# luisdiaz1997/GPzoo

Measured on AMD Instinct MI355X. Metric: ELBO evals/sec (L=32-latent evaluations, all GPUs) at M=2048 inducing, N=200000, L=32 latents/GPU x 1 GPU(s), higher is better.
Workload: dtype f32; 1 GPU; BASELINE configs[2]: Slide-seq-shaped synthetic, N=200000 spots, M=2048, L=32 latents/GPU x 1 GPU(s), matern32, f32; latents_total=32, whitened=True, chunk=0, factor_dtype=f64

## Files before the change

gpzoo_amd/csrc/gemmw.h:

```cpp
#pragma once
#include "common.h"

namespace gpz {

struct Fused1Args {
  const float* Linv; int64_t Mp;
  const float* Z; int64_t M;
  const float* X; int64_t nreal;
  int d, kind, L;
  const float* sigma; const float* ell;
  float* Wt; int64_t ncp;
  const float* muE;
  float* ps_sq; float* ps_mu;
};
bool fused1_supported(int dtype, int kind, int d);
int fused1_launch(const Fused1Args& a, hipStream_t s);

enum WideEpilogue {
  WIDE_STORE_STATS = 0,
  WIDE_STATS = 1,
  WIDE_STORE = 2,
  WIDE_STORE_COLSCALE = 3,
  WIDE_WBAR = 4,
  WIDE_KBAR = 5,
  WIDE_ADD_COLSCALE = 6,
};
struct WideArgs {
  const float* A; const float* B; int64_t Mp, ncp; int L;
  int upper, epilogue;
  float* C; const float* mu;
  float* ps_sq; float* ps_mu;
  const float* colscale; const float* colvec;
  const float* rowvec;
  const float* aux;
  const int32_t* gate;
};
bool wide_product_supported(int64_t Mp, int64_t ncp);
int wide_product_launch(const WideArgs& a, hipStream_t s);

bool wide_nt_supported(int64_t Mp, int64_t K);
int wide_nt_pieces(int64_t Mp, int64_t K, int L);
size_t wide_nt_scratch_floats(int64_t Mp, int64_t K, int L);
size_t wide_nt_vpart_floats(int64_t Mp, int64_t K, int L);
int wide_nt_launch(const float* A, const float* B, float* C, int64_t Mp, int64_t K, int L, hipStream_t s, float* scratch = nullptr,
                   const float* w = nullptr, const int32_t* gate = nullptr, const float* gm = nullptr, float* vpart = nullptr,
                   double* v = nullptr, int64_t v_stride = 0);

}
```

gpzoo_amd/csrc/gemmw.hip:

```cpp
#include "gemmw.h"

#include "cov.h"


#include <cmath>
#include <mutex>
#include <type_traits>
#include <utility>

#ifndef GPZ_W_ABL
#define GPZ_W_ABL 0
#endif

namespace gpz {

typedef float f32x4 __attribute__((ext_vector_type(4)));

enum { WB_MEM = 0, WB_GEN = 1 };
enum { WA_DENSE = 0, WA_LOWER = 1, WA_UPPER = 2 };
enum { WE_STORE_STATS = 0,
       WE_STATS = 1,
       WE_STORE = 2,
       WE_STORE_COLSCALE = 3,
       WE_WBAR = 4,
       WE_KBAR = 5,
       WE_ADD_COLSCALE = 6 };

struct WParams {
  const float* A; int64_t lda, sA0;
  const float* B; int64_t ldb, sB0;
  const float* Z; int64_t MD;
  const float* X; int64_t nreal;
  const float* sigma; const float* ell;
  float* C; int64_t ldc, sC0;
  const float* mu; int64_t sMu;
  float* ps_sq; float* ps_mu; int64_t ncols;
  const float* colscale; const float* colvec; int64_t sCs;
  const float* rowvec; int64_t sRv;
  const float* aux;
  int64_t M;
  int L, nblk, mtw, nt, W, strips;
  int pair, colmajor;
  const int32_t* gate;
};

constexpr int W_BK = 16;

template <int TM, int TN, int BSRC, int D>
struct WLds {
  static constexpr int A_ELEMS = TM * W_BK;
  static constexpr int RPP = 256 / TN;
  static constexpr int PITCH = 256 + (RPP == 2 ? 8 : RPP == 1 ? 4 : 16);
  static constexpr int B_ELEMS = (W_BK / RPP) * PITCH;
  static constexpr int STAGE = A_ELEMS + B_ELEMS;
  static constexpr int ZB = 128 * D;
  static constexpr size_t bytes = sizeof(float) * (2 * STAGE + (BSRC == WB_GEN ? 2 * ZB : 0));
};

template <int TM, int TN, int BSRC, int ATRI, int EPI, int KIND, int D>
__global__ __launch_bounds__(64 * (TM / 128) * (TN / 32)) __attribute__((amdgpu_waves_per_eu(4, 4))) void gemmw_kernel(const WParams p) {
  constexpr int BK = W_BK;
  if (p.gate && *p.gate == 0) return;
  constexpr int WMW = TM / 128, WNW = TN / 32;
  constexpr int NW = WMW * WNW;
  static_assert(NW == 8 || NW == 16, "8 or 16 waves of 128 x 32");
  using G = WLds<TM, TN, BSRC, D>;
  constexpr int RPP = G::RPP, PITCH = G::PITCH;
  extern __shared__ __attribute__((aligned(1024))) char smem_raw[];
  float* const smem = reinterpret_cast<float*>(smem_raw);
  auto sA = [&](int buf) -> float* { return smem + buf * G::STAGE; };
  auto sB = [&](int buf) -> float* { return smem + buf * G::STAGE + G::A_ELEMS; };
  float* const sZ = smem + 2 * G::STAGE;
  auto addrB = [](int k, int n) { return (k / RPP) * PITCH + (k % RPP) * TN + n; };

  int tj, b0, leg_ti[2], nlegs = 1;
  {
    const int bid = blockIdx.x;
    const int x = bid & 7, s = bid >> 3;
    if (BSRC == WB_GEN) {
      const int ug = s / p.W, within = s - ug * p.W;
      const int u = ug * 8 + x;
      const int per_level = p.L * p.strips;
      if (u >= p.mtw * per_level) return;
      const int level = u / per_level, rem = u - level * per_level;
      leg_ti[0] = leg_ti[1] = (ATRI == WA_LOWER) ? p.mtw - 1 - level : level;
      b0 = rem / p.strips;
      tj = (rem - b0 * p.strips) * p.W + within;
    } else {
// ... 257 lines not shown
        for (int g = 0; g < 4; ++g)
#pragma unroll
          for (int ni = 0; ni < 2; ++ni) {
            const float v = acc[mi][ni][g];
            ssq[ni] = __builtin_fmaf(v, v, ssq[ni]);
            if constexpr (EPI == WE_STORE_STATS) smu[ni] = __builtin_fmaf(m4[g], v, smu[ni]);
          }
      }
#pragma unroll
      for (int ni = 0; ni < 2; ++ni) {
        ssq[ni] += __shfl_xor(ssq[ni], 16); ssq[ni] += __shfl_xor(ssq[ni], 32);
        if constexpr (EPI == WE_STORE_STATS) { smu[ni] += __shfl_xor(smu[ni], 16); smu[ni] += __shfl_xor(smu[ni], 32); }
        if (q == 0) {
          const int64_t o = ((int64_t)b0 * p.nblk + db) * p.ncols + ccol0 + ni * 16 + r;
          p.ps_sq[o] = ssq[ni];
          if constexpr (EPI == WE_STORE_STATS) p.ps_mu[o] = smu[ni];
        }
      }
    }
    if constexpr (EPI != WE_STATS) {
      constexpr int LDE = 36;
      static_assert(NW * 16 * LDE <= G::STAGE, "the epilogue strips fit tile buffer 1");
      float* strip = sA(1) + wave * (16 * LDE);
      float* Cg = p.C + b0 * p.sC0 + row0 * p.ldc + ccol0;
      int srow = lane >> 3;
      asm volatile("" : "+v"(srow));
      const int c4 = (lane & 7) * 4;
      float cs[2] = {1.f, 1.f};
      if constexpr (EPI == WE_STORE_COLSCALE) {
#pragma unroll
        for (int ni = 0; ni < 2; ++ni) cs[ni] = p.colscale[b0 * p.sCs + ccol0 + ni * 16 + r];
      }
      f32x4 sc = {0, 0, 0, 0}, cv = {0, 0, 0, 0};
      if constexpr (EPI == WE_WBAR || EPI == WE_KBAR || EPI == WE_ADD_COLSCALE)
        sc = *reinterpret_cast<const f32x4*>(p.colscale + b0 * p.sCs + ccol0 + c4);
      if constexpr (EPI == WE_WBAR || EPI == WE_KBAR)
        cv = *reinterpret_cast<const f32x4*>(p.colvec + b0 * p.sCs + ccol0 + c4);
#pragma unroll
      for (int mi = 0; mi < 8; ++mi) {
#pragma unroll
        for (int ni = 0; ni < 2; ++ni)
#pragma unroll
          for (int g = 0; g < 4; ++g) strip[(4 * q + g) * LDE + ni * 16 + r] = cs[ni] * acc[mi][ni][g];
        __builtin_amdgcn_wave_barrier();
        f32x4 w[2];
        float rv[2];
        if constexpr (EPI == WE_WBAR || EPI == WE_KBAR || EPI == WE_ADD_COLSCALE) {
#pragma unroll
          for (int it = 0; it < 2; ++it) {
            const int64_t row = mi * 16 + it * 8 + srow;
            if constexpr (EPI == WE_WBAR) w[it] = *reinterpret_cast<const f32x4*>(p.aux + b0 * p.sC0 + (row0 + row) * p.ldc + ccol0 + c4);
            if constexpr (EPI == WE_ADD_COLSCALE) w[it] = *reinterpret_cast<const f32x4*>(Cg + (int64_t)row * p.ldc + c4);
            if constexpr (EPI != WE_ADD_COLSCALE) rv[it] = p.rowvec[b0 * p.sRv + row0 + row];
          }
        }
#pragma unroll
        for (int it = 0; it < 2; ++it) {
          const int row = it * 8 + srow;
          f32x4 v = *reinterpret_cast<const f32x4*>(strip + row * LDE + c4);
          if constexpr (EPI == WE_WBAR) {
#pragma unroll
            for (int e = 0; e < 4; ++e) v[e] = v[e] + rv[it] * cv[e] - w[it][e] * sc[e];
          }
          if constexpr (EPI == WE_KBAR) {
#pragma unroll
            for (int e = 0; e < 4; ++e) v[e] = v[e] * sc[e] + rv[it] * cv[e];
          }
          if constexpr (EPI == WE_ADD_COLSCALE) {
#pragma unroll
            for (int e = 0; e < 4; ++e) v[e] = w[it][e] + v[e] * sc[e];
          }
          *reinterpret_cast<f32x4*>(Cg + (int64_t)(mi * 16 + row) * p.ldc + c4) = v;
        }
        __builtin_amdgcn_wave_barrier();
      }
    }
  }
}

struct NTParams {
  const float* A; const float* B; float* C;
  int64_t ld, sAB, ldc, sC;
  int K, nblk, mt, L, T;
  int S, Ks;
  float* part; int64_t sPart;
  const float* w; int64_t sW;
  const int32_t* gate;
  const float* gm; float* vpart;
};

template <int TM, bool WTS>
__global__ __launch_bounds__(TM * 2) __attribute__((amdgpu_waves_per_eu(4, 4))) void gemmw_nt_kernel(const NTParams p) {
  constexpr int BK = W_BK, TN = 128;
  if (p.gate && *p.gate == 0) return;
  constexpr int NW = TM / 32;
  constexpr int A_ELEMS = TM * BK, B_ELEMS = TN * BK, STAGE = A_ELEMS + B_ELEMS;
  extern __shared__ __attribute__((aligned(1024))) char smem_raw[];
  float* const smem = reinterpret_cast<float*>(smem_raw);
  auto sA = [&](int buf) -> float* { return smem + buf * STAGE; };
  auto sB = [&](int buf) -> float* { return smem + buf * STAGE + A_ELEMS; };
  int b0, ti, tj, piece;
  {
    const int nb = (int)gridDim.x, qn = nb >> 3, rem = nb & 7, x = blockIdx.x & 7;
    const int lid0 = x * qn + min(x, rem) + (int)(blockIdx.x >> 3);
    const int grp = lid0 / p.T;
    const int t = lid0 - grp * p.T;
    b0 = grp / p.S;
    piece = grp - b0 * p.S;
    if constexpr (TM == 256) {
      int i = (int)((sqrtf(4.0f * (float)t + 1.0f) - 1.0f) * 0.5f);
      while ((i + 1) * (i + 2) <= t) ++i;
      while (i * (i + 1) > t) --i;
      ti = i; tj = t - i * (i + 1);
    } else {
      int i = (int)((sqrtf(8.0f * (float)t + 1.0f) - 1.0f) * 0.5f);
      while ((i + 1) * (i + 2) / 2 <= t) ++i;
      while (i * (i + 1) / 2 > t) --i;
      ti = i; tj = t - i * (i + 1) / 2;
    }
  }
  const int tid = threadIdx.x, lane = tid & 63;
  const int wave = __builtin_amdgcn_readfirstlane(tid >> 6);
  const int wm = wave >> 2, wn = wave & 3;
  const int r = lane & 15, q = lane >> 4;
  const int Mp = p.nblk * 128;
  const int db = (TM / 128) * ti + wm;
  const bool active = db < p.nblk && tj <= db;
  const bool same = TM == 128 && p.A == p.B && tj == ti;
  typedef __attribute__((address_space(3))) void lds_void;
#if defined(__HIP_DEVICE_COMPILE__)
  const __amdgpu_buffer_rsrc_t a_rsrc = __builtin_amdgcn_make_buffer_rsrc(
      const_cast<float*>(p.A + b0 * p.sAB), 0, (int)(p.ld * Mp * sizeof(float)), 0x00020000);
  const __amdgpu_buffer_rsrc_t b_rsrc = __builtin_amdgcn_make_buffer_rsrc(
      const_cast<float*>(p.B + b0 * p.sAB), 0, (int)(p.ld * Mp * sizeof(float)), 0x00020000);
#endif
  auto gperm = [](int w) { const int t = (w >> 2) & 3; return (((t >> 1) ^ t) & 1) << 1 | (t >> 1); };
  const int voff = ((lane >> 2) * (int)p.ld + (((lane & 3) ^ gperm(lane >> 2)) * 4)) * (int)sizeof(float);
  int a_soff[2], b_soff;
#pragma unroll
  for (int h = 0; h < 2; ++h) {
    int row = ti * TM + (2 * wave + h) * 16;
    while (row >= Mp) row -= 128;
    a_soff[h] = (row * (int)p.ld + piece * p.Ks) * (int)sizeof(float);
  }
  constexpr int NPB = 8 / NW;
  b_soff = ((tj * TN + wave * NPB * 16) * (int)p.ld + piece * p.Ks) * (int)sizeof(float);
  auto stage_load = [&](int buf) __attribute__((always_inline)) {
#if defined(__HIP_DEVICE_COMPILE__)
#pragma unroll
    for (int h = 0; h < 2; ++h) {
      __builtin_amdgcn_raw_ptr_buffer_load_lds(a_rsrc, (lds_void*)(sA(buf) + (2 * wave + h) * 256), 16, voff, a_soff[h], 0, 0);
      a_soff[h] += BK * (int)sizeof(float);
    }
    if (!same) {
#pragma unroll
      for (int h = 0; h < NPB; ++h)
        __builtin_amdgcn_raw_ptr_buffer_load_lds(b_rsrc, (lds_void*)(sB(buf) + (wave * NPB + h) * 256), 16, voff,
                                                 b_soff + h * 16 * (int)p.ld * (int)sizeof(float), 0, 0);
      b_soff += BK * (int)sizeof(float);
    }
#endif
  };
  const float* wk = WTS ? p.w + b0 * p.sW + (int64_t)piece * p.Ks + 4 * (lane >> 4) : nullptr;
  f32x4 wv;
  auto w_load = [&]() __attribute__((always_inline)) {
    if constexpr (WTS) { wv = *reinterpret_cast<const f32x4*>(wk); wk += BK; }
  };
  const int fr_a = (wm * 128 + r) * BK + ((q ^ gperm(r)) * 4);
  const int nk = (min(p.K, (piece + 1) * p.Ks) - piece * p.Ks) / BK;
  const bool split = p.S > 1;
  const bool diag = WTS && p.A == p.B && db == tj && db < p.nblk;
  if (diag) {
    auto diag_path = [&](auto wn_c) __attribute__((always_inline)) {
      constexpr int C0 = decltype(wn_c)::value, C1 = 7 - C0, N0 = 8 - C0, N1 = 8 - C1;
      const bool rd = p.gm != nullptr;
      const float* gk = rd ? p.gm + b0 * p.sW + (int64_t)piece * p.Ks + 4 * (lane >> 4) : nullptr;
      f32x4 gv = f32x4{0, 0, 0, 0};
      float pv0 = 0.f, pv1 = 0.f;
      f32x4 a0[N0], a1[N1];
#pragma unroll
      for (int i = 0; i < N0; ++i) a0[i] = f32x4{0, 0, 0, 0};
#pragma unroll
      for (int i = 0; i < N1; ++i) a1[i] = f32x4{0, 0, 0, 0};
      const int fb_off = r * BK + ((q ^ gperm(r)) * 4) + (same ? -A_ELEMS : 0);
      auto step = [&](int buf, bool more) __attribute__((always_inline)) {
        f32x4 f0 = *reinterpret_cast<const f32x4*>(sB(buf) + fb_off + C0 * 16 * BK);
        f32x4 f1 = *reinterpret_cast<const f32x4*>(sB(buf) + fb_off + C1 * 16 * BK);
        f0 *= wv; f1 *= wv;
        if (more) w_load();
#pragma unroll
        for (int mi = C0; mi < 8; ++mi) {
          const f32x4 fa = *reinterpret_cast<const f32x4*>(sA(buf) + fr_a + mi * 16 * BK);
#pragma unroll
          for (int j = 0; j < 4; ++j) {
            a0[mi - C0] = __builtin_amdgcn_mfma_f32_16x16x4f32(fa[j], f0[j], a0[mi - C0], 0, 0, 0);
            if (mi >= C1) a1[mi >= C1 ? mi - C1 : 0] = __builtin_amdgcn_mfma_f32_16x16x4f32(fa[j], f1[j], a1[mi >= C1 ? mi - C1 : 0], 0, 0, 0);
          }
          if (mi == 2 * C0 || mi == 2 * C0 + 1) {
            if (rd) {
              const f32x4 t = fa * gv;
              if (mi == 2 * C0) pv0 += (t[0] + t[1]) + (t[2] + t[3]); else pv1 += (t[0] + t[1]) + (t[2] + t[3]);
            }
          }
        }
        if (more && rd) { gv = *reinterpret_cast<const f32x4*>(gk); gk += BK; }
      };
      if (rd) { gv = *reinterpret_cast<const f32x4*>(gk); gk += BK; }
      stage_load(0);
      w_load();
      asm volatile("s_waitcnt vmcnt(0)" ::: "memory");
      __syncthreads();
      for (int t = 0; t < nk; t += 2) {
        if (t + 1 < nk) stage_load(1);
        step(0, t + 1 < nk);
        asm volatile("s_waitcnt vmcnt(0)" ::: "memory");
        __syncthreads();
        if (t + 2 < nk) stage_load(0);
        step(1, t + 2 < nk);
        asm volatile("s_waitcnt vmcnt(0)" ::: "memory");
        __syncthreads();
      }
      if (rd) {
        float* vp = p.vpart + ((int64_t)piece * p.L + b0) * Mp + db * 128;
        pv0 += __shfl_xor(pv0, 16); pv0 += __shfl_xor(pv0, 32);
        pv1 += __shfl_xor(pv1, 16); pv1 += __shfl_xor(pv1, 32);
        if (q == 0) { vp[(2 * C0) * 16 + r] = pv0; vp[(2 * C0 + 1) * 16 + r] = pv1; }
      }
      float* Cg = (split ? p.part + piece * p.sPart : p.C) + b0 * p.sC + (int64_t)db * 128 * p.ldc + (int64_t)tj * TN;
      auto put = [&](const f32x4& a, int mi, int c) __attribute__((always_inline)) {
        float* o = Cg + (int64_t)(mi * 16 + 4 * q) * p.ldc + c * 16 + r;
#pragma unroll
        for (int g = 0; g < 4; ++g) o[g * p.ldc] = split ? a[g] : o[g * p.ldc] + a[g];
      };
#pragma unroll
      for (int mi = C0; mi < 8; ++mi) put(a0[mi - C0], mi, C0);
#pragma unroll
      for (int mi = C1; mi < 8; ++mi) put(a1[mi - C1], mi, C1);
    };
    switch (wn) {
      case 0: diag_path(std::integral_constant<int, 0>{}); break;
      case 1: diag_path(std::integral_constant<int, 1>{}); break;
      case 2: diag_path(std::integral_constant<int, 2>{}); break;
      default: diag_path(std::integral_constant<int, 3>{}); break;
    }
    return;
  }
  f32x4 acc[8][2];
#pragma unroll
  for (int mi = 0; mi < 8; ++mi)
#pragma unroll
    for (int ni = 0; ni < 2; ++ni) acc[mi][ni] = f32x4{0, 0, 0, 0};
  const int fr_b = (wn * 32 + r) * BK + ((q ^ gperm(r)) * 4) + (same ? -A_ELEMS : 0);
  auto mma_step = [&](int buf, bool more) __attribute__((always_inline)) {
    f32x4 fb[2];
#pragma unroll
    for (int ni = 0; ni < 2; ++ni) {
      fb[ni] = *reinterpret_cast<const f32x4*>(sB(buf) + fr_b + ni * 16 * BK);
      if constexpr (WTS) fb[ni] *= wv;
    }
    if (more) w_load();
#pragma unroll
    for (int half = 0; half < 2; ++half) {
      f32x4 fa[4];
#pragma unroll
      for (int m = 0; m < 4; ++m) fa[m] = *reinterpret_cast<const f32x4*>(sA(buf) + fr_a + (half * 4 + m) * 16 * BK);
#pragma unroll
      for (int j = 0; j < 4; ++j)
#pragma unroll
        for (int m = 0; m < 4; ++m)
#pragma unroll
          for (int ni = 0; ni < 2; ++ni)
            acc[half * 4 + m][ni] = __builtin_amdgcn_mfma_f32_16x16x4f32(fa[m][j], fb[ni][j], acc[half * 4 + m][ni], 0, 0, 0);
    }
  };
  stage_load(0);
  w_load();
  asm volatile("s_waitcnt vmcnt(0)" ::: "memory");
  __syncthreads();
  if (active) {
    for (int t = 0; t < nk; t += 2) {
      if (t + 1 < nk) stage_load(1);
      mma_step(0, t + 1 < nk);
      asm volatile("s_waitcnt vmcnt(0)" ::: "memory");
      __syncthreads();
      if (t + 2 < nk) stage_load(0);
      mma_step(1, t + 2 < nk);
      asm volatile("s_waitcnt vmcnt(0)" ::: "memory");
      __syncthreads();
    }
  } else {
    for (int t = 0; t < nk; t += 2) {
      if (t + 1 < nk) stage_load(1);
      asm volatile("s_waitcnt vmcnt(0)" ::: "memory");
      __syncthreads();
      if (t + 2 < nk) stage_load(0);
      asm volatile("s_waitcnt vmcnt(0)" ::: "memory");
      __syncthreads();
    }
    return;
  }
  constexpr int LDE = 36;
  float* strip = smem + wave * (32 * LDE);
  float* Cg = (split ? p.part + piece * p.sPart : p.C) + b0 * p.sC + (int64_t)db * 128 * p.ldc + (int64_t)tj * TN + wn * 32;
  const int srow = lane >> 3, c4 = (lane & 7) * 4;
#pragma unroll
  for (int pass = 0; pass < 4; ++pass) {
#pragma unroll
    for (int mm = 0; mm < 2; ++mm)
#pragma unroll
      for (int ni = 0; ni < 2; ++ni)
#pragma unroll
        for (int g = 0; g < 4; ++g) strip[(mm * 16 + 4 * q + g) * LDE + ni * 16 + r] = acc[pass * 2 + mm][ni][g];
    __builtin_amdgcn_wave_barrier();
    f32x4 cin[4];
#pragma unroll
    for (int it = 0; it < 4; ++it)
      cin[it] = split ? f32x4{0, 0, 0, 0} : *reinterpret_cast<const f32x4*>(Cg + (int64_t)(pass * 32 + it * 8 + srow) * p.ldc + c4);
#pragma unroll
    for (int it = 0; it < 4; ++it) {
      const int row = it * 8 + srow;
      const f32x4 v = *reinterpret_cast<const f32x4*>(strip + row * LDE + c4);
      *reinterpret_cast<f32x4*>(Cg + (int64_t)(pass * 32 + row) * p.ldc + c4) = cin[it] + v;
    }
    __builtin_amdgcn_wave_barrier();
  }
}
// ... 64 lines not shown
  p.L = a.L; p.nblk = (int)(a.Mp / 128); p.mtw = (int)((a.Mp + TM - 1) / TM); p.nt = (int)(a.ncp / TN);
  int strips = (p.nt + 31) / 32;
  const int want = (32 + p.mtw * p.L - 1) / (p.mtw * p.L);
  if (strips < want) strips = want < p.nt ? want : p.nt;
  p.W = (p.nt + strips - 1) / strips;
  p.strips = (p.nt + p.W - 1) / p.W;
  const int64_t units = (int64_t)p.mtw * p.L * p.strips;
  const int64_t nblocks = (units + 7) / 8 * 8 * p.W;
#define GPZ_W1(KIND, D) return launch_wide(gemmw_kernel<TM, TN, WB_GEN, WA_LOWER, WE_STORE_STATS, KIND, D>, \
                                           WLds<TM, TN, WB_GEN, D>::bytes, p, nblocks, s, 1024)
  if (a.kind == GPZ_KERNEL_MATERN32) { if (a.d == 2) GPZ_W1(1, 2); GPZ_W1(1, 1); }
  if (a.kind == GPZ_KERNEL_MATERN12) { if (a.d == 2) GPZ_W1(4, 2); GPZ_W1(4, 1); }
  if (a.kind == GPZ_KERNEL_MATERN52) { if (a.d == 2) GPZ_W1(5, 2); GPZ_W1(5, 1); }
  if (a.d == 2) GPZ_W1(0, 2);
  GPZ_W1(0, 1);
#undef GPZ_W1
}

bool wide_product_supported(int64_t Mp, int64_t ncp) {
  return Mp % 128 == 0 && ncp % 128 == 0 && Mp * Mp * 4 < (1ll << 31) && Mp * ncp * 4 < (1ll << 31);
}

template <int TM, int TN>
static int wide_product_launch_t(const WideArgs& a, hipStream_t s) {
  WParams p = {};
  p.A = a.A; p.lda = a.Mp; p.sA0 = a.Mp * a.Mp;
  p.B = a.B; p.ldb = a.ncp; p.sB0 = a.Mp * a.ncp;
  p.C = a.C; p.ldc = a.ncp; p.sC0 = a.Mp * a.ncp;
  p.mu = a.mu; p.sMu = a.Mp;
  p.ps_sq = a.ps_sq; p.ps_mu = a.ps_mu; p.ncols = a.ncp; p.M = a.Mp;
  p.colscale = a.colscale; p.colvec = a.colvec; p.sCs = a.ncp; p.rowvec = a.rowvec; p.sRv = a.Mp; p.aux = a.aux;
  p.gate = a.gate;
  p.L = a.L; p.nblk = (int)(a.Mp / 128); p.mtw = (int)((a.Mp + TM - 1) / TM); p.nt = (int)((a.ncp + TN - 1) / TN);
  constexpr int WMAX = 4096 / TN;
  int strips = (p.nt + WMAX - 1) / WMAX;
  const int want = (8 + p.L - 1) / p.L;
  if (strips < want) strips = want < p.nt ? want : p.nt;
  p.strips = strips;
  p.W = (p.nt + strips - 1) / strips;
  const int64_t units = (int64_t)p.L * p.strips;
  const int64_t paired = (units + 7) / 8 * 8 * ((p.mtw + 1) / 2) * p.W;
  p.pair = p.colmajor = paired >= 4 * 512;
  const int64_t nblocks = p.pair ? paired : (units + 7) / 8 * 8 * p.mtw * p.W;
  constexpr size_t lds = WLds<TM, TN, WB_MEM, 1>::bytes;
#define GPZ_WM(ATRI, EPI) return launch_wide(gemmw_kernel<TM, TN, WB_MEM, ATRI, EPI, 0, 1>, lds, p, nblocks, s)
  switch (a.epilogue) {
    case WIDE_STORE_STATS:
      GPZ_REQUIRE(!a.upper && a.C && a.mu && a.ps_sq && a.ps_mu, "wide product: store + statistics is the lower-triangular product and needs C, mu and both slabs");
      GPZ_WM(WA_LOWER, WE_STORE_STATS);
    case WIDE_STATS:
      GPZ_REQUIRE(a.upper && a.ps_sq, "wide product: statistics only is the upper-triangular product");
      GPZ_WM(WA_UPPER, WE_STATS);
    case WIDE_STORE:
      GPZ_REQUIRE(a.upper && a.C, "wide product: the plain store is built for the upper-triangular product");
      GPZ_WM(WA_UPPER, WE_STORE);
    case WIDE_STORE_COLSCALE:
      GPZ_REQUIRE(a.upper && a.C && a.colscale, "wide product: the column-scaled store is the upper-triangular product and needs the factors");
      GPZ_WM(WA_UPPER, WE_STORE_COLSCALE);
    case WIDE_WBAR:
      GPZ_REQUIRE(!a.upper && a.C && a.colscale && a.colvec && a.rowvec && a.aux, "wide product: the W-bar epilogue needs its operands");
      GPZ_WM(WA_LOWER, WE_WBAR);
    case WIDE_KBAR:
      GPZ_REQUIRE(a.upper == 2 && a.C && a.colscale && a.colvec && a.rowvec, "wide product: the K-bar epilogue is the dense product and needs its vectors");
      GPZ_WM(WA_DENSE, WE_KBAR);
    case WIDE_ADD_COLSCALE:
      GPZ_REQUIRE(a.upper == 1 && a.C && a.colscale, "wide product: the accumulating column-scaled store is the upper-triangular product");
      GPZ_WM(WA_UPPER, WE_ADD_COLSCALE);
    default: break;
  }
#undef GPZ_WM
  GPZ_REQUIRE(false, "wide product: unknown epilogue %d", a.epilogue);
}

int wide_product_launch(const WideArgs& a, hipStream_t s) {
  GPZ_REQUIRE(wide_product_supported(a.Mp, a.ncp) && a.L > 0, "wide product: bad extents");
  return wide_product_launch_t<128, 256>(a, s);
}

bool wide_nt_supported(int64_t Mp, int64_t K) {
  return Mp % 128 == 0 && K % 128 == 0 && K > 0 && Mp * K * 4 < (1ll << 31);
}

static bool nt_small_tiles(int64_t nblk) { return nblk <= 4; }
static int64_t nt_tiles(int64_t nblk) {
  if (nt_small_tiles(nblk)) return nblk * (nblk + 1) / 2;
  const int64_t mt = (nblk + 1) / 2;
  return mt * (mt + 1) - (nblk & 1);
}

int wide_nt_pieces(int64_t Mp, int64_t K, int L) {
  const int64_t tiles = nt_tiles(Mp / 128) * L;
  if (tiles >= 384) {
    const double r = (double)tiles / 512.0;
    int best = 1;
    double best_cost = 1e30;
    for (int S = 1; S <= 4; ++S) {
      if (S > 1 && K / S < 2048) break;
      const double rounds = r * S, cost = std::ceil(rounds - 1e-9) / rounds * (1.0 + 0.015 * (S - 1));
      if (cost < best_cost - 1e-9) { best_cost = cost; best = S; }
    }
    return best;
  }
  int64_t S = (nt_small_tiles(Mp / 128) ? 1024 : 512) / tiles;
  S = std::min<int64_t>(S, K / 1024);
  S = std::min<int64_t>(S, 16);
  return (int)std::max<int64_t>(S, 1);
}

size_t wide_nt_vpart_floats(int64_t Mp, int64_t K, int L) { return (size_t)wide_nt_pieces(Mp, K, L) * L * Mp; }

size_t wide_nt_scratch_floats(int64_t Mp, int64_t K, int L) {
  const int S = wide_nt_pieces(Mp, K, L);
  return S > 1 ? (size_t)S * L * Mp * Mp : 0;
}

int wide_nt_launch(const float* A, const float* B, float* C, int64_t Mp, int64_t K, int L, hipStream_t s, float* scratch,
                   const float* w, const int32_t* gate, const float* gm, float* vpart, double* v, int64_t v_stride) {
  GPZ_REQUIRE(A && B && C && wide_nt_supported(Mp, K) && L > 0, "wide A B^T: bad arguments");
  GPZ_REQUIRE(!gm || (w && vpart && v && A == B), "wide A B^T: the row products A gm need weights, A == B and their buffers");
  NTParams p;
  p.w = w; p.sW = K; p.gate = gate; p.gm = gm; p.vpart = vpart;
  p.A = A; p.B = B; p.C = C; p.ld = K; p.sAB = Mp * K; p.ldc = Mp; p.sC = Mp * Mp;
  p.K = (int)K; p.nblk = (int)(Mp / 128); p.mt = (p.nblk + 1) / 2; p.L = L;
  const bool small = nt_small_tiles(p.nblk);
  p.T = (int)nt_tiles(p.nblk);
  int S = scratch ? wide_nt_pieces(Mp, K, L) : 1;
  p.Ks = (int)(((K + S - 1) / S + 31) / 32 * 32);
  S = (int)((K + p.Ks - 1) / p.Ks);
  p.S = S; p.part = scratch; p.sPart = (int64_t)L * Mp * Mp;
  const int64_t nblocks = (int64_t)p.T * L * S;
  GPZ_REQUIRE(nblocks > 0 && nblocks < (1ll << 31), "wide A B^T: bad grid");
  if (small) {
    constexpr size_t lds = sizeof(float) * 2 * (128 + 128) * W_BK;
    if (w) hipLaunchKernelGGL((gemmw_nt_kernel<128, true>), dim3((unsigned)nblocks), dim3(256), lds, s, p);
    else hipLaunchKernelGGL((gemmw_nt_kernel<128, false>), dim3((unsigned)nblocks), dim3(256), lds, s, p);
  } else {
    constexpr size_t lds = sizeof(float) * 2 * (256 + 128) * W_BK;
    if (w) hipLaunchKernelGGL((gemmw_nt_kernel<256, true>), dim3((unsigned)nblocks), dim3(512), lds, s, p);
    else hipLaunchKernelGGL((gemmw_nt_kernel<256, false>), dim3((unsigned)nblocks), dim3(512), lds, s, p);
  }
  GPZ_LAUNCH_OK();
  if (S > 1) {
    const int64_t total4 = (int64_t)L * Mp * Mp / 4;
    hipLaunchKernelGGL(nt_reduce_kernel, dim3((unsigned)((total4 + 255) / 256)), dim3(256), 0, s, C, scratch, S, p.sPart, (int)Mp, total4, gate, (int)(w != nullptr && A == B));
    GPZ_LAUNCH_OK();
  }
  if (gm) {
    const int64_t LM = (int64_t)L * Mp;
    hipLaunchKernelGGL(nt_vsum_kernel, dim3((unsigned)((LM + 255) / 256)), dim3(256), 0, s, vpart, S, LM, v, Mp, v_stride);
    GPZ_LAUNCH_OK();
  }
  return 0;
}

}
```

Measured before the change: 2.637 ELBO evals/s.

## Add symmetric diagonal-tile schedule for weighted A·Aᵀ wide NT kernel

For the weighted symmetric case (A == B with weights) on large tiles, the grid now schedules mt*mt tiles. Each diagonal 256-row tile is computed by one block that loads only A and forms the lower triangle of the 256x256 block, where the old schedule used separate 256x128 tiles. This avoids redundant B loads and the upper-triangle MFMA work on diagonal blocks, and changes the split-K piece count to match the new tile count. It adds a large per-wave specialized path that raises register pressure, and the old schedule stays available through an environment variable.

```diff
diff --git a/gpzoo_amd/csrc/gemmw.h b/gpzoo_amd/csrc/gemmw.h
--- a/gpzoo_amd/csrc/gemmw.h
+++ b/gpzoo_amd/csrc/gemmw.h
@@ -39,7 +39,7 @@
 int wide_product_launch(const WideArgs& a, hipStream_t s);
 
 bool wide_nt_supported(int64_t Mp, int64_t K);
-int wide_nt_pieces(int64_t Mp, int64_t K, int L);
+int wide_nt_pieces(int64_t Mp, int64_t K, int L, bool sym = false);
 size_t wide_nt_scratch_floats(int64_t Mp, int64_t K, int L);
 size_t wide_nt_vpart_floats(int64_t Mp, int64_t K, int L);
 int wide_nt_launch(const float* A, const float* B, float* C, int64_t Mp, int64_t K, int L, hipStream_t s, float* scratch = nullptr,
diff --git a/gpzoo_amd/csrc/gemmw.hip b/gpzoo_amd/csrc/gemmw.hip
--- a/gpzoo_amd/csrc/gemmw.hip
+++ b/gpzoo_amd/csrc/gemmw.hip
@@ -4,6 +4,8 @@
 
 
 #include <cmath>
+#include <cstdlib>
+#include <cstring>
 #include <mutex>
 #include <type_traits>
 #include <utility>
@@ -432,6 +434,7 @@
   const float* w; int64_t sW;
   const int32_t* gate;
   const float* gm; float* vpart;
+  int dtiles;
 };
 
 template <int TM, bool WTS>
@@ -445,6 +448,7 @@
   auto sA = [&](int buf) -> float* { return smem + buf * STAGE; };
   auto sB = [&](int buf) -> float* { return smem + buf * STAGE + A_ELEMS; };
   int b0, ti, tj, piece;
+  bool dtile = false;
   {
     const int nb = (int)gridDim.x, qn = nb >> 3, rem = nb & 7, x = blockIdx.x & 7;
     const int lid0 = x * qn + min(x, rem) + (int)(blockIdx.x >> 3);
@@ -452,7 +456,18 @@
     const int t = lid0 - grp * p.T;
     b0 = grp / p.S;
     piece = grp - b0 * p.S;
-    if constexpr (TM == 256) {
+    if (TM == 256 && WTS && p.dtiles) {
+      if (t < p.mt) {
+        ti = t; tj = 2 * t;
+        dtile = 2 * t + 1 < p.nblk;
+      } else {
+        const int u = t - p.mt;
+        int i = (int)((sqrtf(4.0f * (float)u + 1.0f) + 1.0f) * 0.5f);
+        while (i * (i + 1) <= u) ++i;
+        while (i * (i - 1) > u) --i;
+        ti = i; tj = u - i * (i - 1);
+      }
+    } else if constexpr (TM == 256) {
       int i = (int)((sqrtf(4.0f * (float)t + 1.0f) - 1.0f) * 0.5f);
       while ((i + 1) * (i + 2) <= t) ++i;
       while (i * (i + 1) > t) --i;
@@ -497,7 +512,7 @@
       __builtin_amdgcn_raw_ptr_buffer_load_lds(a_rsrc, (lds_void*)(sA(buf) + (2 * wave + h) * 256), 16, voff, a_soff[h], 0, 0);
       a_soff[h] += BK * (int)sizeof(float);
     }
-    if (!same) {
+    if (!same && !dtile) {
 #pragma unroll
       for (int h = 0; h < NPB; ++h)
         __builtin_amdgcn_raw_ptr_buffer_load_lds(b_rsrc, (lds_void*)(sB(buf) + (wave * NPB + h) * 256), 16, voff,
@@ -506,14 +521,121 @@
     }
 #endif
   };
-  const float* wk = WTS ? p.w + b0 * p.sW + (int64_t)piece * p.Ks + 4 * (lane >> 4) : nullptr;
+  const float* wk = WTS ? p.w + b0 * p.sW + (int64_t)piece * p.Ks : nullptr;
+  const unsigned klane = 4 * (unsigned)(lane >> 4);
   f32x4 wv;
   auto w_load = [&]() __attribute__((always_inline)) {
-    if constexpr (WTS) { wv = *reinterpret_cast<const f32x4*>(wk); wk += BK; }
+    if constexpr (WTS) { wv = *reinterpret_cast<const f32x4*>(wk + klane); wk += BK; }
   };
   const int fr_a = (wm * 128 + r) * BK + ((q ^ gperm(r)) * 4);
   const int nk = (min(p.K, (piece + 1) * p.Ks) - piece * p.Ks) / BK;
   const bool split = p.S > 1;
+  if constexpr (TM == 256 && WTS) {
+    if (dtile) {
+      auto dtile_path = [&](auto w_c) __attribute__((always_inline)) {
+        constexpr int C0 = decltype(w_c)::value, C1 = 15 - C0, N0 = 16 - C0, N1 = 16 - C1;
+        const bool rd = p.gm != nullptr;
+        const float* gk = rd ? p.gm + b0 * p.sW + (int64_t)piece * p.Ks : nullptr;
+        f32x4 gv = f32x4{0, 0, 0, 0};
+        float pv0 = 0.f, pv1 = 0.f;
+        f32x4 a0[N0], a1[N1];
+#pragma unroll
+        for (int i = 0; i < N0; ++i) a0[i] = f32x4{0, 0, 0, 0};
+#pragma unroll
+        for (int i = 0; i < N1; ++i) a1[i] = f32x4{0, 0, 0, 0};
+        const int fr = r * BK + ((q ^ gperm(r)) * 4);
+        auto step = [&](int buf, bool more) __attribute__((always_inline)) {
+          f32x4 f0 = *reinterpret_cast<const f32x4*>(sA(buf) + fr + C0 * 16 * BK);
+          f32x4 f1 = *reinterpret_cast<const f32x4*>(sA(buf) + fr + C1 * 16 * BK);
+          f0 *= wv; f1 *= wv;
+          if (more) w_load();
+#pragma unroll
+          for (int mi = C0; mi < 16; ++mi) {
+            const f32x4 fa = *reinterpret_cast<const f32x4*>(sA(buf) + fr + mi * 16 * BK);
+#pragma unroll
+            for (int j = 0; j < 4; ++j) {
+              a0[mi - C0] = __builtin_amdgcn_mfma_f32_16x16x4f32(fa[j], f0[j], a0[mi - C0], 0, 0, 0);
+              if (mi >= C1) a1[mi >= C1 ? mi - C1 : 0] = __builtin_amdgcn_mfma_f32_16x16x4f32(fa[j], f1[j], a1[mi >= C1 ? mi - C1 : 0], 0, 0, 0);
+            }
+            if (mi == 2 * C0 || mi == 2 * C0 + 1) {
+              if (rd) {
+                const f32x4 t = fa * gv;
+                if (mi == 2 * C0) pv0 += (t[0] + t[1]) + (t[2] + t[3]); else pv1 += (t[0] + t[1]) + (t[2] + t[3]);
+              }
+            }
+          }
+          if (more && rd) { gv = *reinterpret_cast<const f32x4*>(gk + klane); gk += BK; }
+        };
+        if (rd) { gv = *reinterpret_cast<const f32x4*>(gk + klane); gk += BK; }
+        stage_load(0);
+        w_load();
+        asm volatile("s_waitcnt vmcnt(0)" ::: "memory");
+        __syncthreads();
+        for (int t = 0; t < nk; t += 2) {
+          if (t + 1 < nk) stage_load(1);
+          step(0, t + 1 < nk);
+          asm volatile("s_waitcnt vmcnt(0)" ::: "memory");
+          __syncthreads();
+          if (t + 2 < nk) stage_load(0);
+          step(1, t + 2 < nk);
+          asm volatile("s_waitcnt vmcnt(0)" ::: "memory");
+          __syncthreads();
+        }
+        if (rd) {
+          float* vp = p.vpart + ((int64_t)piece * p.L + b0) * Mp + ti * 256;
+          pv0 += __shfl_xor(pv0, 16); pv0 += __shfl_xor(pv0, 32);
+          pv1 += __shfl_xor(pv1, 16); pv1 += __shfl_xor(pv1, 32);
+          if (q == 0) { vp[(2 * C0) * 16 + r] = pv0; vp[(2 * C0 + 1) * 16 + r] = pv1; }
+        }
+#if defined(__HIP_DEVICE_COMPILE__)
+        const __amdgpu_buffer_rsrc_t c_rsrc = __builtin_amdgcn_make_buffer_rsrc(
+            (split ? p.part + piece * p.sPart : p.C) + b0 * p.sC, 0, (int)(p.ldc * Mp * sizeof(float)), 0x00020000);
+        const int ldcb = (int)p.ldc * (int)sizeof(float);
+        const int lo = 4 * q * ldcb + r * (int)sizeof(float);
+        const int so = ti * 256 * ldcb + ti * 256 * (int)sizeof(float);
+        auto put_col = [&](const f32x4* a, auto c_c, auto split_c) __attribute__((always_inline)) {
+          constexpr int CC = decltype(c_c)::value;
+#pragma unroll
+          for (int m0 = CC; m0 < 16; m0 += 4) {
+            float cin[4][4];
+#pragma unroll
+            for (int m = 0; m < 4; ++m)
+#pragma unroll
+              for (int g = 0; g < 4; ++g)
+                if (!decltype(split_c)::value && m0 + m < 16)
+                  cin[m][g] = __builtin_bit_cast(float, __builtin_amdgcn_raw_buffer_load_b32(c_rsrc, lo, so + ((m0 + m) * 16 + g) * ldcb + CC * 64, 0));
+#pragma unroll
+            for (int m = 0; m < 4; ++m)
+#pragma unroll
+              for (int g = 0; g < 4; ++g)
+                if (m0 + m < 16) {
+                  const float v = decltype(split_c)::value ? a[m0 + m - CC][g] : cin[m][g] + a[m0 + m - CC][g];
+                  __builtin_amdgcn_raw_buffer_store_b32(__builtin_bit_cast(unsigned, v), c_rsrc, lo, so + ((m0 + m) * 16 + g) * ldcb + CC * 64, 0);
+                }
+          }
+        };
+        if (split) {
+          put_col(a0, std::integral_constant<int, C0>{}, std::true_type{});
+          put_col(a1, std::integral_constant<int, C1>{}, std::true_type{});
+        } else {
+          put_col(a0, std::integral_constant<int, C0>{}, std::false_type{});
+          put_col(a1, std::integral_constant<int, C1>{}, std::false_type{});
+        }
+#endif
+      };
+      switch (wave) {
+        case 0: dtile_path(std::integral_constant<int, 0>{}); break;
+        case 1: dtile_path(std::integral_constant<int, 1>{}); break;
+        case 2: dtile_path(std::integral_constant<int, 2>{}); break;
+        case 3: dtile_path(std::integral_constant<int, 3>{}); break;
+        case 4: dtile_path(std::integral_constant<int, 4>{}); break;
+        case 5: dtile_path(std::integral_constant<int, 5>{}); break;
+        case 6: dtile_path(std::integral_constant<int, 6>{}); break;
+        default: dtile_path(std::integral_constant<int, 7>{}); break;
+      }
+      return;
+    }
+  }
   const bool diag = WTS && p.A == p.B && db == tj && db < p.nblk;
   if (diag) {
     auto diag_path = [&](auto wn_c) __attribute__((always_inline)) {
@@ -817,14 +939,22 @@
 }
 
 static bool nt_small_tiles(int64_t nblk) { return nblk <= 4; }
-static int64_t nt_tiles(int64_t nblk) {
+
+static bool nt_diag_tiles() {
+  const char* e = getenv("GPZ_NT_SCHEDULE");
+  return !(e && !strcmp(e, "blocks"));
+}
+
+static bool nt_sym_tiles(int64_t nblk, bool sym) { return sym && !nt_small_tiles(nblk) && nt_diag_tiles(); }
+static int64_t nt_tiles(int64_t nblk, bool sym_tiles) {
   if (nt_small_tiles(nblk)) return nblk * (nblk + 1) / 2;
   const int64_t mt = (nblk + 1) / 2;
+  if (sym_tiles) return mt * mt;
   return mt * (mt + 1) - (nblk & 1);
 }
 
-int wide_nt_pieces(int64_t Mp, int64_t K, int L) {
-  const int64_t tiles = nt_tiles(Mp / 128) * L;
+int wide_nt_pieces(int64_t Mp, int64_t K, int L, bool sym) {
+  const int64_t tiles = nt_tiles(Mp / 128, nt_sym_tiles(Mp / 128, sym)) * L;
   if (tiles >= 384) {
     const double r = (double)tiles / 512.0;
     int best = 1;
@@ -842,10 +972,12 @@
   return (int)std::max<int64_t>(S, 1);
 }
 
-size_t wide_nt_vpart_floats(int64_t Mp, int64_t K, int L) { return (size_t)wide_nt_pieces(Mp, K, L) * L * Mp; }
+static int nt_pieces_max(int64_t Mp, int64_t K, int L) { return std::max(wide_nt_pieces(Mp, K, L, false), wide_nt_pieces(Mp, K, L, true)); }
+
+size_t wide_nt_vpart_floats(int64_t Mp, int64_t K, int L) { return (size_t)nt_pieces_max(Mp, K, L) * L * Mp; }
 
 size_t wide_nt_scratch_floats(int64_t Mp, int64_t K, int L) {
-  const int S = wide_nt_pieces(Mp, K, L);
+  const int S = nt_pieces_max(Mp, K, L);
   return S > 1 ? (size_t)S * L * Mp * Mp : 0;
 }
 
@@ -858,8 +990,10 @@
   p.A = A; p.B = B; p.C = C; p.ld = K; p.sAB = Mp * K; p.ldc = Mp; p.sC = Mp * Mp;
   p.K = (int)K; p.nblk = (int)(Mp / 128); p.mt = (p.nblk + 1) / 2; p.L = L;
   const bool small = nt_small_tiles(p.nblk);
-  p.T = (int)nt_tiles(p.nblk);
-  int S = scratch ? wide_nt_pieces(Mp, K, L) : 1;
+  const bool sym = w && A == B;
+  p.dtiles = nt_sym_tiles(p.nblk, sym);
+  p.T = (int)nt_tiles(p.nblk, p.dtiles);
+  int S = scratch ? wide_nt_pieces(Mp, K, L, sym) : 1;
   p.Ks = (int)(((K + S - 1) / S + 31) / 32 * 32);
   S = (int)((K + p.Ks - 1) / p.Ks);
   p.S = S; p.part = scratch; p.sPart = (int64_t)L * Mp * Mp;
```

After: 2.626 ELBO evals/s. Within noise of the previous version (-0.4%).

## Pair adjacent diagonal blocks into one tile for symmetric weighted NT product

Applied to the files above, without the earlier changes.

For the symmetric weighted A·Aᵀ case with 256-row tiles, tiles are remapped so that each diagonal tile covers two consecutive 128-row diagonal blocks and loads only A. This shrinks the tile grid from mt(mt+1) to mt², so fewer blocks redo or skip the redundant upper half. The diagonal path is templated on NB blocks, with per-block accumulators and sched barriers. In exchange it raises register pressure in the diagonal path and changes the split-K piece selection.

```diff
diff --git a/gpzoo_amd/csrc/gemmw.h b/gpzoo_amd/csrc/gemmw.h
--- a/gpzoo_amd/csrc/gemmw.h
+++ b/gpzoo_amd/csrc/gemmw.h
@@ -39,7 +39,7 @@
 int wide_product_launch(const WideArgs& a, hipStream_t s);
 
 bool wide_nt_supported(int64_t Mp, int64_t K);
-int wide_nt_pieces(int64_t Mp, int64_t K, int L);
+int wide_nt_pieces(int64_t Mp, int64_t K, int L, bool sym);
 size_t wide_nt_scratch_floats(int64_t Mp, int64_t K, int L);
 size_t wide_nt_vpart_floats(int64_t Mp, int64_t K, int L);
 int wide_nt_launch(const float* A, const float* B, float* C, int64_t Mp, int64_t K, int L, hipStream_t s, float* scratch = nullptr,
diff --git a/gpzoo_amd/csrc/gemmw.hip b/gpzoo_amd/csrc/gemmw.hip
--- a/gpzoo_amd/csrc/gemmw.hip
+++ b/gpzoo_amd/csrc/gemmw.hip
@@ -427,6 +427,7 @@
   const float* A; const float* B; float* C;
   int64_t ld, sAB, ldc, sC;
   int K, nblk, mt, L, T;
+  int sym;
   int S, Ks;
   float* part; int64_t sPart;
   const float* w; int64_t sW;
@@ -445,6 +446,7 @@
   auto sA = [&](int buf) -> float* { return smem + buf * STAGE; };
   auto sB = [&](int buf) -> float* { return smem + buf * STAGE + A_ELEMS; };
   int b0, ti, tj, piece;
+  bool dunit = false;
   {
     const int nb = (int)gridDim.x, qn = nb >> 3, rem = nb & 7, x = blockIdx.x & 7;
     const int lid0 = x * qn + min(x, rem) + (int)(blockIdx.x >> 3);
@@ -453,10 +455,23 @@
     b0 = grp / p.S;
     piece = grp - b0 * p.S;
     if constexpr (TM == 256) {
-      int i = (int)((sqrtf(4.0f * (float)t + 1.0f) - 1.0f) * 0.5f);
-      while ((i + 1) * (i + 2) <= t) ++i;
-      while (i * (i + 1) > t) --i;
-      ti = i; tj = t - i * (i + 1);
+      if (WTS && p.sym) {
+        if (t < p.mt) {
+          ti = t; tj = 2 * t;
+          dunit = 2 * t + 1 < p.nblk;
+        } else {
+          const int u = t - p.mt;
+          int i = (int)((sqrtf(4.0f * (float)u + 1.0f) + 1.0f) * 0.5f);
+          while (i * (i + 1) <= u) ++i;
+          while (i * (i - 1) > u) --i;
+          ti = i; tj = u - i * (i - 1);
+        }
+      } else {
+        int i = (int)((sqrtf(4.0f * (float)t + 1.0f) - 1.0f) * 0.5f);
+        while ((i + 1) * (i + 2) <= t) ++i;
+        while (i * (i + 1) > t) --i;
+        ti = i; tj = t - i * (i + 1);
+      }
     } else {
       int i = (int)((sqrtf(8.0f * (float)t + 1.0f) - 1.0f) * 0.5f);
       while ((i + 1) * (i + 2) / 2 <= t) ++i;
@@ -471,7 +486,7 @@
   const int Mp = p.nblk * 128;
   const int db = (TM / 128) * ti + wm;
   const bool active = db < p.nblk && tj <= db;
-  const bool same = TM == 128 && p.A == p.B && tj == ti;
+  const bool same = (TM == 128 && p.A == p.B && tj == ti) || dunit;
   typedef __attribute__((address_space(3))) void lds_void;
 #if defined(__HIP_DEVICE_COMPILE__)
   const __amdgpu_buffer_rsrc_t a_rsrc = __builtin_amdgcn_make_buffer_rsrc(
@@ -506,51 +521,59 @@
     }
 #endif
   };
-  const float* wk = WTS ? p.w + b0 * p.sW + (int64_t)piece * p.Ks + 4 * (lane >> 4) : nullptr;
+  const float* wk = WTS ? p.w + b0 * p.sW + (int64_t)piece * p.Ks : nullptr;
+  const int kq = 4 * (lane >> 4);
   f32x4 wv;
   auto w_load = [&]() __attribute__((always_inline)) {
-    if constexpr (WTS) { wv = *reinterpret_cast<const f32x4*>(wk); wk += BK; }
+    if constexpr (WTS) { wv = *reinterpret_cast<const f32x4*>(wk + kq); wk += BK; }
   };
   const int fr_a = (wm * 128 + r) * BK + ((q ^ gperm(r)) * 4);
   const int nk = (min(p.K, (piece + 1) * p.Ks) - piece * p.Ks) / BK;
   const bool split = p.S > 1;
   const bool diag = WTS && p.A == p.B && db == tj && db < p.nblk;
   if (diag) {
-    auto diag_path = [&](auto wn_c) __attribute__((always_inline)) {
-      constexpr int C0 = decltype(wn_c)::value, C1 = 7 - C0, N0 = 8 - C0, N1 = 8 - C1;
+    auto diag_path = [&](auto wn_c, auto nb_c) __attribute__((always_inline)) {
+      constexpr int C0 = decltype(wn_c)::value, C1 = 7 - C0, N0 = 8 - C0, N1 = 8 - C1, NB = decltype(nb_c)::value;
       const bool rd = p.gm != nullptr;
-      const float* gk = rd ? p.gm + b0 * p.sW + (int64_t)piece * p.Ks + 4 * (lane >> 4) : nullptr;
+      const float* gk = rd ? p.gm + b0 * p.sW + (int64_t)piece * p.Ks : nullptr;
       f32x4 gv = f32x4{0, 0, 0, 0};
-      float pv0 = 0.f, pv1 = 0.f;
-      f32x4 a0[N0], a1[N1];
-#pragma unroll
-      for (int i = 0; i < N0; ++i) a0[i] = f32x4{0, 0, 0, 0};
-#pragma unroll
-      for (int i = 0; i < N1; ++i) a1[i] = f32x4{0, 0, 0, 0};
+      float pv0[NB], pv1[NB];
+      f32x4 a0[NB][N0], a1[NB][N1];
+#pragma unroll
+      for (int b = 0; b < NB; ++b) {
+        pv0[b] = pv1[b] = 0.f;
+#pragma unroll
+        for (int i = 0; i < N0; ++i) a0[b][i] = f32x4{0, 0, 0, 0};
+#pragma unroll
+        for (int i = 0; i < N1; ++i) a1[b][i] = f32x4{0, 0, 0, 0};
+      }
       const int fb_off = r * BK + ((q ^ gperm(r)) * 4) + (same ? -A_ELEMS : 0);
       auto step = [&](int buf, bool more) __attribute__((always_inline)) {
-        f32x4 f0 = *reinterpret_cast<const f32x4*>(sB(buf) + fb_off + C0 * 16 * BK);
-        f32x4 f1 = *reinterpret_cast<const f32x4*>(sB(buf) + fb_off + C1 * 16 * BK);
-        f0 *= wv; f1 *= wv;
-        if (more) w_load();
-#pragma unroll
-        for (int mi = C0; mi < 8; ++mi) {
-          const f32x4 fa = *reinterpret_cast<const f32x4*>(sA(buf) + fr_a + mi * 16 * BK);
-#pragma unroll
-          for (int j = 0; j < 4; ++j) {
-            a0[mi - C0] = __builtin_amdgcn_mfma_f32_16x16x4f32(fa[j], f0[j], a0[mi - C0], 0, 0, 0);
-            if (mi >= C1) a1[mi >= C1 ? mi - C1 : 0] = __builtin_amdgcn_mfma_f32_16x16x4f32(fa[j], f1[j], a1[mi >= C1 ? mi - C1 : 0], 0, 0, 0);
-          }
-          if (mi == 2 * C0 || mi == 2 * C0 + 1) {
-            if (rd) {
+#pragma unroll
+        for (int b = 0; b < NB; ++b) {
+          f32x4 f0 = *reinterpret_cast<const f32x4*>(sB(buf) + fb_off + (b * 128 + C0 * 16) * BK);
+          f32x4 f1 = *reinterpret_cast<const f32x4*>(sB(buf) + fb_off + (b * 128 + C1 * 16) * BK);
+          f0 *= wv; f1 *= wv;
+          if (b == NB - 1 && more) w_load();
+#pragma unroll
+          for (int mi = C0; mi < 8; ++mi) {
+            const f32x4 fa = *reinterpret_cast<const f32x4*>(sA(buf) + fr_a + (b * 128 + mi * 16) * BK);
+#pragma unroll
+            for (int j = 0; j < 4; ++j) {
+              a0[b][mi - C0] = __builtin_amdgcn_mfma_f32_16x16x4f32(fa[j], f0[j], a0[b][mi - C0], 0, 0, 0);
+              if (mi >= C1) a1[b][mi >= C1 ? mi - C1 : 0] = __builtin_amdgcn_mfma_f32_16x16x4f32(fa[j], f1[j], a1[b][mi >= C1 ? mi - C1 : 0], 0, 0, 0);
+            }
+            if (mi == 2 * C0 || mi == 2 * C0 + 1) {
               const f32x4 t = fa * gv;
-              if (mi == 2 * C0) pv0 += (t[0] + t[1]) + (t[2] + t[3]); else pv1 += (t[0] + t[1]) + (t[2] + t[3]);
+              if (mi == 2 * C0) { pv0[b] += (t[0] + t[1]) + (t[2] + t[3]); asm volatile("" : "+v"(pv0[b])); }
+              else { pv1[b] += (t[0] + t[1]) + (t[2] + t[3]); asm volatile("" : "+v"(pv1[b])); }
             }
+            if constexpr (NB == 2) __builtin_amdgcn_sched_barrier(0);
           }
         }
-        if (more && rd) { gv = *reinterpret_cast<const f32x4*>(gk); gk += BK; }
+        if (more && rd) { gv = *reinterpret_cast<const f32x4*>(gk + kq); gk += BK; }
       };
-      if (rd) { gv = *reinterpret_cast<const f32x4*>(gk); gk += BK; }
+      if (rd) { gv = *reinterpret_cast<const f32x4*>(gk + kq); gk += BK; }
       stage_load(0);
       w_load();
       asm volatile("s_waitcnt vmcnt(0)" ::: "memory");
@@ -565,28 +588,47 @@
         asm volatile("s_waitcnt vmcnt(0)" ::: "memory");
         __syncthreads();
       }
-      if (rd) {
-        float* vp = p.vpart + ((int64_t)piece * p.L + b0) * Mp + db * 128;
-        pv0 += __shfl_xor(pv0, 16); pv0 += __shfl_xor(pv0, 32);
-        pv1 += __shfl_xor(pv1, 16); pv1 += __shfl_xor(pv1, 32);
-        if (q == 0) { vp[(2 * C0) * 16 + r] = pv0; vp[(2 * C0 + 1) * 16 + r] = pv1; }
-      }
-      float* Cg = (split ? p.part + piece * p.sPart : p.C) + b0 * p.sC + (int64_t)db * 128 * p.ldc + (int64_t)tj * TN;
-      auto put = [&](const f32x4& a, int mi, int c) __attribute__((always_inline)) {
-        float* o = Cg + (int64_t)(mi * 16 + 4 * q) * p.ldc + c * 16 + r;
-#pragma unroll
-        for (int g = 0; g < 4; ++g) o[g * p.ldc] = split ? a[g] : o[g * p.ldc] + a[g];
-      };
-#pragma unroll
-      for (int mi = C0; mi < 8; ++mi) put(a0[mi - C0], mi, C0);
-#pragma unroll
-      for (int mi = C1; mi < 8; ++mi) put(a1[mi - C1], mi, C1);
+      int le = lane;
+      asm volatile("" : "+v"(le));
+      const int r = le & 15, q = le >> 4;
+#pragma unroll
+      for (int b = 0; b < NB; ++b) {
+        if (rd) {
+          float* vp = p.vpart + ((int64_t)piece * p.L + b0) * Mp + (db + b) * 128;
+          float s0 = pv0[b], s1 = pv1[b];
+          s0 += __shfl_xor(s0, 16); s0 += __shfl_xor(s0, 32);
+          s1 += __shfl_xor(s1, 16); s1 += __shfl_xor(s1, 32);
+          if (q == 0) { vp[(2 * C0) * 16 + r] = s0; vp[(2 * C0 + 1) * 16 + r] = s1; }
+        }
+        float* Cg = (split ? p.part + piece * p.sPart : p.C) + b0 * p.sC + (int64_t)(db + b) * 128 * p.ldc + (int64_t)(tj + b) * TN;
+        auto put = [&](const f32x4& a, int mi, int c) __attribute__((always_inline)) {
+          float* o = Cg + (int64_t)(mi * 16 + 4 * q) * p.ldc + c * 16 + r;
+#pragma unroll
+          for (int g = 0; g < 4; ++g) o[g * p.ldc] = split ? a[g] : o[g * p.ldc] + a[g];
+        };
+#pragma unroll
+        for (int mi = C0; mi < 8; ++mi) put(a0[b][mi - C0], mi, C0);
+#pragma unroll
+        for (int mi = C1; mi < 8; ++mi) put(a1[b][mi - C1], mi, C1);
+      }
     };
-    switch (wn) {
-      case 0: diag_path(std::integral_constant<int, 0>{}); break;
-      case 1: diag_path(std::integral_constant<int, 1>{}); break;
-      case 2: diag_path(std::integral_constant<int, 2>{}); break;
-      default: diag_path(std::integral_constant<int, 3>{}); break;
+    using std::integral_constant;
+    if (TM == 256 && dunit) {
+      if constexpr (TM == 256) {
+        switch (wn) {
+          case 0: diag_path(integral_constant<int, 0>{}, integral_constant<int, 2>{}); break;
+          case 1: diag_path(integral_constant<int, 1>{}, integral_constant<int, 2>{}); break;
+          case 2: diag_path(integral_constant<int, 2>{}, integral_constant<int, 2>{}); break;
+          default: diag_path(integral_constant<int, 3>{}, integral_constant<int, 2>{}); break;
+        }
+      }
+    } else {
+      switch (wn) {
+        case 0: diag_path(integral_constant<int, 0>{}, integral_constant<int, 1>{}); break;
+        case 1: diag_path(integral_constant<int, 1>{}, integral_constant<int, 1>{}); break;
+        case 2: diag_path(integral_constant<int, 2>{}, integral_constant<int, 1>{}); break;
+        default: diag_path(integral_constant<int, 3>{}, integral_constant<int, 1>{}); break;
+      }
     }
     return;
   }
@@ -817,14 +859,15 @@
 }
 
 static bool nt_small_tiles(int64_t nblk) { return nblk <= 4; }
-static int64_t nt_tiles(int64_t nblk) {
+static int64_t nt_tiles(int64_t nblk, bool sym) {
   if (nt_small_tiles(nblk)) return nblk * (nblk + 1) / 2;
   const int64_t mt = (nblk + 1) / 2;
+  if (sym) return mt * mt;
   return mt * (mt + 1) - (nblk & 1);
 }
 
-int wide_nt_pieces(int64_t Mp, int64_t K, int L) {
-  const int64_t tiles = nt_tiles(Mp / 128) * L;
+int wide_nt_pieces(int64_t Mp, int64_t K, int L, bool sym) {
+  const int64_t tiles = nt_tiles(Mp / 128, sym) * L;
   if (tiles >= 384) {
     const double r = (double)tiles / 512.0;
     int best = 1;
@@ -842,10 +885,10 @@
   return (int)std::max<int64_t>(S, 1);
 }
 
-size_t wide_nt_vpart_floats(int64_t Mp, int64_t K, int L) { return (size_t)wide_nt_pieces(Mp, K, L) * L * Mp; }
+size_t wide_nt_vpart_floats(int64_t Mp, int64_t K, int L) { return (size_t)wide_nt_pieces(Mp, K, L, true) * L * Mp; }
 
 size_t wide_nt_scratch_floats(int64_t Mp, int64_t K, int L) {
-  const int S = wide_nt_pieces(Mp, K, L);
+  const int S = std::max(wide_nt_pieces(Mp, K, L, false), wide_nt_pieces(Mp, K, L, true));
   return S > 1 ? (size_t)S * L * Mp * Mp : 0;
 }
 
@@ -858,8 +901,10 @@
   p.A = A; p.B = B; p.C = C; p.ld = K; p.sAB = Mp * K; p.ldc = Mp; p.sC = Mp * Mp;
   p.K = (int)K; p.nblk = (int)(Mp / 128); p.mt = (p.nblk + 1) / 2; p.L = L;
   const bool small = nt_small_tiles(p.nblk);
-  p.T = (int)nt_tiles(p.nblk);
-  int S = scratch ? wide_nt_pieces(Mp, K, L) : 1;
+  const bool sym = w != nullptr && A == B;
+  p.sym = sym && !small;
+  p.T = (int)nt_tiles(p.nblk, sym);
+  int S = scratch ? wide_nt_pieces(Mp, K, L, sym) : 1;
   p.Ks = (int)(((K + S - 1) / S + 31) / 32 * 32);
   S = (int)((K + p.Ks - 1) / p.Ks);
   p.S = S; p.part = scratch; p.sPart = (int64_t)L * Mp * Mp;
@@ -877,7 +922,7 @@
   GPZ_LAUNCH_OK();
   if (S > 1) {
     const int64_t total4 = (int64_t)L * Mp * Mp / 4;
-    hipLaunchKernelGGL(nt_reduce_kernel, dim3((unsigned)((total4 + 255) / 256)), dim3(256), 0, s, C, scratch, S, p.sPart, (int)Mp, total4, gate, (int)(w != nullptr && A == B));
+    hipLaunchKernelGGL(nt_reduce_kernel, dim3((unsigned)((total4 + 255) / 256)), dim3(256), 0, s, C, scratch, S, p.sPart, (int)Mp, total4, gate, (int)sym);
     GPZ_LAUNCH_OK();
   }
   if (gm) {
```

Measured after the change: 2.635 ELBO evals/s before, 2.632 ELBO evals/s after. No clear change (-0.1%).
